# SunJiamei/LRP-ImageCaptioning

Measured on AMD Instinct MI355X. Metric: LRP heatmaps/sec (per predicted token) VGG16+adaptive-attn, 224x224, higher is better.
Workload: dtype bf16x3; 1 GPU; batch=32 synthetic 224x224 per GPU, VGG16 + adaptive-attention, LRP per-token heat-maps, 10 words/caption, V=10000 (BASELINE configs[1]); parallelism=image-sharded x1, RCCL weight broadcast, reverse_walk_precision=bf16x3, handles_per_gpu=2

## Files before the change

lrp-imagecaptioning_amd/csrc/common.h:

```cpp
#pragma once
#include <hip/hip_runtime.h>
#include <atomic>
#include <cstdarg>
#include <cstdio>
#include <cstdlib>
#include <string>
#include <vector>

#include "../../include/lrp_hip.h"

namespace lrp {

inline std::atomic<unsigned long long> g_launch_count{0};
#undef hipLaunchKernelGGL
#define hipLaunchKernelGGL(kernelName, numBlocks, numThreads, memPerBlock, streamId, ...)                  \
  do {                                                                                                    \
    ::lrp::g_launch_count.fetch_add(1, std::memory_order_relaxed);                                       \
    kernelName<<<(numBlocks), (numThreads), (memPerBlock), (streamId)>>>(__VA_ARGS__);                   \
  } while (0)

std::string& last_error_ref();

struct Switches {
  int conv_halo = 1;
  int conv_breg = 1;
  int conv_small = 1;
  int conv_mid = 1;
  int epi_fast = 1;
  int up2_pw = 1;
  int tile_order = 1;
  int fwd_emit = 1;
  int fwd_il = 1;
  int img_fused = 1;
  int up2_compact = 1;
  int img_fold = 1;
  int pool_fused = 1;
  int sparse_pool = 0;
  void load() {
    *this = Switches();
    auto rd = [](const char* name, int& v) { if (const char* e = getenv(name)) v = atoi(e); };
    rd("LRP_CONV_HALO", conv_halo); rd("LRP_CONV_BREG", conv_breg); rd("LRP_CONV_SMALL", conv_small);
    rd("LRP_CONV_MID", conv_mid); rd("LRP_EPI_FAST", epi_fast); rd("LRP_UP2_PW", up2_pw); rd("LRP_TILE_ORDER", tile_order);
    rd("LRP_FWD_EMIT", fwd_emit); rd("LRP_FWD_IL", fwd_il); rd("LRP_IMG_FUSED", img_fused); rd("LRP_UP2_COMPACT", up2_compact);
    rd("LRP_IMG_FOLD", img_fold); rd("LRP_SPARSE_POOL", sparse_pool); rd("LRP_POOL_FUSED", pool_fused);
  }
};
inline Switches& sw() {
  static Switches s = [] { Switches t; t.load(); return t; }();
  return s;
}

inline int fail(int code, const char* fmt, ...) {
  char buf[512];
  va_list ap;
  va_start(ap, fmt);
  vsnprintf(buf, sizeof(buf), fmt, ap);
  va_end(ap);
  last_error_ref() = buf;
  return code;
}

#define LRP_HIP_CHECK(expr)                                                                     \
  do {                                                                                          \
    hipError_t _e = (expr);                                                                     \
    if (_e != hipSuccess)                                                                       \
      return ::lrp::fail(LRP_ERR_HIP, "%s failed: %s (%s:%d)", #expr, hipGetErrorString(_e), \
                         __FILE__, __LINE__);                                                   \
  } while (0)

#define LRP_TRY(expr)         \
  do {                        \
    int _rc = (expr);         \
    if (_rc != LRP_OK) return _rc; \
  } while (0)

struct DevBuf {
  void* p = nullptr;
  size_t bytes = 0;
  bool owned = true;
  DevBuf() = default;
  DevBuf(const DevBuf&) = delete;
  DevBuf& operator=(const DevBuf&) = delete;
  DevBuf(DevBuf&& o) noexcept : p(o.p), bytes(o.bytes), owned(o.owned) { o.p = nullptr; o.bytes = 0; o.owned = true; }
  DevBuf& operator=(DevBuf&& o) noexcept {
    if (this != &o) { release(); p = o.p; bytes = o.bytes; owned = o.owned; o.p = nullptr; o.bytes = 0; o.owned = true; }
    return *this;
  }
  ~DevBuf() { release(); }
  void release() {
    if (p && owned) (void)hipFree(p);
    p = nullptr;
    bytes = 0;
    owned = true;
  }
  void view_of(const DevBuf& arena, size_t offset, size_t n) {
    release();
    p = static_cast<char*>(arena.p) + offset;
    bytes = n;
    owned = false;
  }
  int alloc(size_t n, int64_t* total) {
    release();
    if (n == 0) n = 16;
    hipError_t e = hipMalloc(&p, n);
    if (e != hipSuccess) {
      p = nullptr;
      (void)hipGetLastError();
      return fail(LRP_ERR_NOMEM, "device memory: hipMalloc(%zu bytes) failed: %s", n, hipGetErrorString(e));
    }
    bytes = n;
    if (total) *total += (int64_t)n;
    return LRP_OK;
  }
  template <typename T>
  T* as() const { return reinterpret_cast<T*>(p); }
};

}
```

lrp-imagecaptioning_amd/csrc/conv_sparse.h:

```cpp
#pragma once
#include "cnn_kernels.h"
#include "conv_igemm.h"

namespace lrp {

typedef __bf16 bf16x16 __attribute__((ext_vector_type(16)));
typedef unsigned u32x2 __attribute__((ext_vector_type(2)));

struct SparseArgs {
  const float* sc;
  const unsigned* idxp;
  const float* wsp;
  const float* gate;
  float* out;
  const int* row2img;
  int NB, Hp, Wp, C, N;
  int cols_t, m_tiles, n_tiles;
  int out_plain;
  int diag;
};

constexpr int SP_TW = 14, SP_TH = 18, SP_PITCH = SP_TW + 2;
constexpr int SP_NENT = (SP_TH + 2) * SP_PITCH;
constexpr int SP_PENT = SP_NENT + 1;
constexpr int SP_SUB = SP_PENT * 16;
constexpr int SP_ABUF = 3 * SP_SUB;
constexpr int SP_SUBPIECES = (SP_PENT + 63) / 64;
constexpr int SP_APIECES = 3 * SP_SUBPIECES;
constexpr int SP_ASLOTS = (SP_APIECES + 7) / 8;
constexpr int SP_BSTAGE = 32768, SP_NSTAGE = 4;
constexpr int SP_LDS = SP_NSTAGE * SP_BSTAGE + 2 * SP_ABUF + 128;
static_assert(SP_LDS <= 160 * 1024, "LDS");
static_assert(SP_PENT >= 64, "a DMA piece is 64 windows");

__host__ __device__ inline int sparse_slot_tap(int q, int group, int slot) {
  const int qy = q >> 1, qx = q & 1, sy = qy ? 1 : -1, sx = qx ? 1 : -1;
  int dy, dx;
  if (group == 0) { dy = (slot >> 1) - qy; dx = (slot & 1) - qx; }
  else if (group == 1) {
    if (slot < 2) { dy = slot - qy; dx = sx; }
    else if (slot == 2) { dy = sy; dx = sx; }
    else return -1;
  } else {
    if (slot < 2) { dy = sy; dx = slot - qx; }
    else return -1;
  }
  return 3 * (dy + 1) + (dx + 1);
}

__global__ __launch_bounds__(256) void conv_sparse_index_kernel(const unsigned char* __restrict__ pos, unsigned* __restrict__ idxp, size_t n_sets,
                                                                int HW, int C) {
  for (size_t i = (size_t)blockIdx.x * 256 + threadIdx.x; i < n_sets * 4; i += (size_t)gridDim.x * 256) {
    const int q = (int)(i & 3);
    const size_t set = i >> 2;
    const u32x2 pp = *reinterpret_cast<const u32x2*>(pos + set * 8);
    const unsigned qxm = (q & 1) ? 0x01010101u : 0u, qym = (q >> 1) ? 0x01010101u : 0u;
    unsigned word[4][2];
#pragma unroll
    for (int d = 0; d < 2; ++d) {
      const unsigned P = pp[d];
      const unsigned px = P & 0x01010101u, py = (P >> 1) & 0x01010101u;
      const unsigned mh = px ^ qxm, mv = py ^ qym;
      const unsigned nmh = mh ^ 0x01010101u, nmv = mv ^ 0x01010101u;
      word[0][d] = P | ((P ^ 0x01010101u) << 2);
      word[1][d] = py | nmh | (nmh << 1);
      word[2][d] = (0x02020202u | ((mh & mv) ^ 0x01010101u)) << 2;
      word[3][d] = (px & mv) | (nmv << 1) | 0x0C0C0C0Cu;
    }
    unsigned h0[4], h1[4];
#pragma unroll
    for (int pl = 0; pl < 4; ++pl) {
      const unsigned t0 = word[pl][0] | (word[pl][0] >> 4), t1 = word[pl][1] | (word[pl][1] >> 4);
      h0[pl] = (t0 & 0xFFu) | (((t0 >> 16) & 0xFFu) << 8);
      h1[pl] = (t1 & 0xFFu) | (((t1 >> 16) & 0xFFu) << 8);
    }
    const u32x4 iw = {h0[0] | (h0[1] << 16), h0[2] | (h0[3] << 16), h1[0] | (h1[1] << 16), h1[2] | (h1[3] << 16)};
    const int spw = C >> 3;
    const size_t win = set / spw;
    const int sw = (int)(set - win * spw), chunk = sw >> 1, s2 = sw & 1;
    const size_t img = win / HW, pix = win - img * HW;
    reinterpret_cast<u32x4*>(idxp)[((((img * 4 + q) * (C >> 4) + chunk) * HW + pix) << 1) + s2] = iw;
  }
}

__global__ __launch_bounds__(256) void conv_sparse_pairs_kernel(const float* __restrict__ sc, float* __restrict__ scp, size_t n_sets, int HW, int C) {
  for (size_t i = (size_t)blockIdx.x * 256 + threadIdx.x; i < n_sets; i += (size_t)gridDim.x * 256) {
    float v[8];
    *reinterpret_cast<f32x4*>(v) = *reinterpret_cast<const f32x4*>(sc + i * 8);
    *reinterpret_cast<f32x4*>(v + 4) = *reinterpret_cast<const f32x4*>(sc + i * 8 + 4);
    const int spw = C >> 3;
    const size_t win = i / spw;
    const int sw = (int)(i - win * spw), chunk = sw >> 1, s2 = sw & 1;
    const size_t n = win / HW, pix = win - n * HW;
    split8_store(v, scp + ((((n * (C >> 4) + chunk) * HW + pix) << 1) + s2) * 8);
  }
}

__global__ __launch_bounds__(256) void conv_sparse_relayout_kernel(const float* __restrict__ pairs, float* __restrict__ scp, size_t n_sets, int HW, int C) {
  for (size_t i = (size_t)blockIdx.x * 256 + threadIdx.x; i < n_sets; i += (size_t)gridDim.x * 256) {
    const u32x4 hi = *reinterpret_cast<const u32x4*>(pairs + i * 8), lo = *reinterpret_cast<const u32x4*>(pairs + i * 8 + 4);
    const int spw = C >> 3;
    const size_t win = i / spw;
    const int sw_ = (int)(i - win * spw), chunk = sw_ >> 1, s2 = sw_ & 1;
    const size_t n = win / HW, pix = win - n * HW;
    float* dst = scp + ((((n * (C >> 4) + chunk) * HW + pix) << 1) + s2) * 8;
    *reinterpret_cast<u32x4*>(dst) = hi;
    *reinterpret_cast<u32x4*>(dst + 4) = lo;
  }
}

__global__ __launch_bounds__(256) void conv_sparse_pack_kernel(const float* __restrict__ wb, float* __restrict__ wsp, int N, int C, int CPo,
                                                               int n_tiles) {
  const size_t total = (size_t)4 * n_tiles * (C / 16) * 6 * 2 * 2 * 256;
  for (size_t i = (size_t)blockIdx.x * 256 + threadIdx.x; i < total; i += (size_t)gridDim.x * 256) {
    const int col = (int)(i & 255);
    size_t r = i >> 8;
    const int part = (int)(r & 1); r >>= 1;
    const int half = (int)(r & 1); r >>= 1;
    const int step = (int)(r % 6); r /= 6;
    const int chunk = (int)(r % (C / 16)); r /= (C / 16);
    const int nt = (int)(r % n_tiles);
    const int q = (int)(r / n_tiles);
    const int ci = nt * 256 + col;
    bf16x8 hi, lo;
#pragma unroll
    for (int e = 0; e < 8; ++e) {
      const int k32 = 16 * half + 8 * part + e, cb = k32 >> 2, slot = k32 & 3;
      const int ch8 = 4 * ((cb >> 1) & 1) + 2 * (cb >> 2) + (cb & 1);
      const int co = chunk * 16 + (step & 1) * 8 + ch8;
      const int tap = sparse_slot_tap(q, step >> 1, slot);
      const float v = (tap >= 0 && ci < N && co < C) ? wb[(size_t)ci * 9 * CPo + (size_t)tap * CPo + co] : 0.f;
      hi[e] = (__bf16)v;
      lo[e] = (__bf16)(v - (float)hi[e]);
    }
    const size_t sbase = ((((size_t)q * n_tiles + nt) * (C / 16) + chunk) * 6 + step) * (SP_BSTAGE / 16);
    u32x4* dst = reinterpret_cast<u32x4*>(wsp);
    dst[sbase + ((0 * 2 + half) * 2 + part) * 256 + col] = __builtin_bit_cast(u32x4, hi);
    dst[sbase + ((1 * 2 + half) * 2 + part) * 256 + col] = __builtin_bit_cast(u32x4, lo);
  }
}

__global__ __launch_bounds__(512, 2) void conv_sparse_kernel(SparseArgs a) {
#if defined(__HIP_DEVICE_COMPILE__)
  __shared__ __attribute__((aligned(16))) unsigned char lds[SP_LDS];
  const int tid = threadIdx.x, lane = tid & 63, wave = tid >> 6, wm = wave >> 2, wn = wave & 3;
  const int l31 = lane & 31, half = lane >> 5;
  const int per_class = a.m_tiles * a.n_tiles;
  const int q = blockIdx.x / per_class, rem = blockIdx.x - q * per_class;
  const int nt = rem / a.m_tiles, mt = rem - nt * a.m_tiles;
  const int qy = q >> 1, qx = q & 1, sy = qy ? 1 : -1, sx = qx ? 1 : -1;
  const int tyt = mt / a.cols_t, txt = mt - tyt * a.cols_t;
  const int Y0 = tyt * SP_TH, x0 = txt * SP_TW;
  const int Hp = a.Hp, Wp = a.Wp, C = a.C, N = a.N, H = 2 * Hp, W = 2 * Wp;
  const int nys = a.NB * Hp;
  const int n0 = nt * 256;
  const float inv_Hp = 1.0f / (float)Hp;
  auto divmod = [](int x, int d, float inv, int& qq, int& r) {
    qq = (int)(((float)x + 0.5f) * inv);
    r = x - qq * d;
    if (r < 0) { --qq; r += d; } else if (r >= d) { ++qq; r -= d; }
  };
  unsigned char* Bs = lds;
  unsigned char* As = lds + SP_NSTAGE * SP_BSTAGE;

  auto chunk0 = [&](int e) { return e * 16 + half * 8; };
  int e_own[4], e_h[4], e_v[4], e_d[4];
#pragma unroll
  for (int i = 0; i < 4; ++i) {
    const int r = (wm * 4 + i) * 32 + l31;
    const int ty = r / SP_TW, tx = r - ty * SP_TW;
    const int Ys = Y0 + ty, wx = x0 + tx;
    int n_, wy;
    divmod(Ys, Hp, inv_Hp, n_, wy);
    const bool ok = r < SP_TH * SP_TW && Ys < nys && wx < Wp;
    const bool okh = ok && wx + sx >= 0 && wx + sx < Wp, okv = ok && wy + sy >= 0 && wy + sy < Hp;
    const int e = (ty + 1) * SP_PITCH + tx + 1;
    e_own[i] = chunk0(ok ? e : SP_NENT);
    e_h[i] = chunk0(okh ? e + sx : SP_NENT);
    e_v[i] = chunk0(okv ? e + sy * SP_PITCH : SP_NENT);
    e_d[i] = chunk0(okh && okv ? e + sy * SP_PITCH + sx : SP_NENT);
  }

  typedef __attribute__((address_space(3))) void* lptr_t;
  constexpr int RSRC_FLAGS = 0x00020000;
  const int nchunks = C >> 4, nsteps = nchunks * 6;
  const __amdgpu_buffer_rsrc_t rsB = __builtin_amdgcn_make_buffer_rsrc(
      (void*)(reinterpret_cast<const unsigned char*>(a.wsp) + ((size_t)q * a.n_tiles + nt) * (size_t)nsteps * SP_BSTAGE), 0, nsteps * SP_BSTAGE, RSRC_FLAGS);
  const int wave_s = __builtin_amdgcn_readfirstlane(wave);
  auto fire_b = [&](int step, int stage) {
#pragma unroll
    for (int p = 0; p < 4; ++p)
      __builtin_amdgcn_raw_ptr_buffer_load_lds(rsB, (lptr_t)(Bs + stage * SP_BSTAGE + (wave_s * 4 + p) * 1024), 16, lane * 16,
                                               step * SP_BSTAGE + (wave_s * 4 + p) * 1024, 0, 0);
  };

  int* imgtab = reinterpret_cast<int*>(As + 2 * SP_ABUF);
  if (tid < SP_TH + 2) {
    const int Ys = Y0 - 1 + tid;
    int n_, wy;
    divmod(Ys >= 0 && Ys < nys ? Ys : 0, Hp, inv_Hp, n_, wy);
    imgtab[tid] = a.row2img ? a.row2img[n_] : n_;
  }
  const __amdgpu_buffer_rsrc_t rsS = __builtin_amdgcn_make_buffer_rsrc((void*)a.sc, 0, 0x7FFFFFFF, RSRC_FLAGS);
  const __amdgpu_buffer_rsrc_t rsI = __builtin_amdgcn_make_buffer_rsrc((void*)a.idxp, 0, 0x7FFFFFFF, RSRC_FLAGS);
  constexpr int OOB = (int)0x80000000;
  auto fire_a = [&](int slot, int set8, int abuf) {
    int wv = wave_s, ln = lane;
    asm volatile("" : "+s"(wv), "+v"(ln));
    int pj = wv + 8 * slot;
    if (pj >= SP_APIECES) pj = SP_APIECES - 1;
    const int pl = pj / SP_SUBPIECES, jp = pj - pl * SP_SUBPIECES;
    const int first = jp * 64 < SP_PENT - 64 ? jp * 64 : SP_PENT - 64;
    const int e = first + ln;
    const int hy = e >> 4, hx = e & 15;
    const int Ys = Y0 - 1 + hy, wx = x0 - 1 + hx;
    const bool ok = e < SP_NENT && Ys >= 0 && Ys < nys && wx >= 0 && wx < Wp;
    int n_, wy;
    divmod(ok ? Ys : 0, Hp, inv_Hp, n_, wy);
    const int chunk = set8 >> 1, s = set8 & 1;
    int vo;
    if (pl < 2) {
      vo = ((((n_ * (C >> 4) + chunk) * Hp + wy) * Wp + wx) << 6) + s * 32 + pl * 16;
    } else {
      const int img = imgtab[ok ? hy : 0];
      vo = (((((img * 4 + q) * (C >> 4) + chunk) * Hp + wy) * Wp + wx) << 5) + s * 16;
    }
    __builtin_amdgcn_raw_ptr_buffer_load_lds(pl < 2 ? rsS : rsI, (lptr_t)(As + abuf * SP_ABUF + pl * SP_SUB + first * 16), 16, ok ? vo : OOB,
                                             0, 0, 0);
  };
  auto fire_set = [&](int set8, int abuf) {
#pragma unroll
    for (int sl = 0; sl < SP_ASLOTS; ++sl) fire_a(sl, set8, abuf);
  };

  const int nsteps2 = nchunks * 6;
  auto bsrc = [&](int chunk, int t6) { return chunk * 6 + 2 * (t6 % 3) + t6 / 3; };
  __syncthreads();
  fire_set(0, 0);
  if (nchunks * 2 > 1) fire_set(1, 1);
  fire_b(bsrc(0, 0), 0);
  fire_b(bsrc(0, 1), 1);
  asm volatile("s_waitcnt vmcnt(0)" ::: "memory");
  __syncthreads();

  f32x16 acc[4][2];
#pragma unroll
  for (int i = 0; i < 4; ++i)
#pragma unroll
    for (int j = 0; j < 2; ++j)
#pragma unroll
      for (int r = 0; r < 16; ++r) acc[i][j][r] = 0.f;

  const int bcol = (wn * 64 + l31) * 16 + half * 8192;
  auto expand = [](u32x2 x) -> bf16x8 {
    const u32x4 r = {x[0] & 0xFFFFu, x[0] >> 16, x[1] & 0xFFFFu, x[1] >> 16};
    return __builtin_bit_cast(bf16x8, r);
  };
  auto pairup = [](u32x2 h, u32x2 d) -> bf16x8 {
    const u32x4 r = {__builtin_amdgcn_perm(d[0], h[0], 0x05040100u), __builtin_amdgcn_perm(d[0], h[0], 0x07060302u),
                     __builtin_amdgcn_perm(d[1], h[1], 0x05040100u), __builtin_amdgcn_perm(d[1], h[1], 0x07060302u)};
    return __builtin_bit_cast(bf16x8, r);
  };
  auto ld8 = [](const unsigned char* p) { return *reinterpret_cast<const u32x2*>(p); };
  auto ld2 = [](const unsigned char* p) { return (unsigned)*reinterpret_cast<const unsigned short*>(p); };
  struct BF { bf16x16 h[2], l[2]; };
  auto load_b = [&](BF& b, const unsigned char* Bb) {
#pragma unroll
    for (int j = 0; j < 2; ++j) {
      const unsigned char* bp = Bb + j * 512;
      const bf16x8 h0 = *reinterpret_cast<const bf16x8*>(bp), h1 = *reinterpret_cast<const bf16x8*>(bp + 4096);
      const bf16x8 l0 = *reinterpret_cast<const bf16x8*>(bp + 16384), l1 = *reinterpret_cast<const bf16x8*>(bp + 16384 + 4096);
      b.h[j] = __builtin_shufflevector(h0, h1, 0, 1, 2, 3, 4, 5, 6, 7, 8, 9, 10, 11, 12, 13, 14, 15);
      b.l[j] = __builtin_shufflevector(l0, l1, 0, 1, 2, 3, 4, 5, 6, 7, 8, 9, 10, 11, 12, 13, 14, 15);
    }
  };
  auto kstep = [&](const unsigned char* Ab, int grp, const BF& b) {
    const unsigned char* Ah = Ab;
    const unsigned char* Al = Ab + SP_SUB;
    const unsigned char* Ai = Ab + 2 * SP_SUB;
#pragma unroll
    for (int i = 0; i < 4; ++i) {
      bf16x8 vh, vl;
      int ix;
      if (grp == 1) {
        const int oh = e_h[i], od = e_d[i];
        vh = pairup(ld8(Ah + oh), ld8(Ah + od));
        vl = pairup(ld8(Al + oh), ld8(Al + od));
        ix = (int)(ld2(Ai + oh + 2) | ld2(Ai + od + 4));
      } else {
        const int oo = grp == 0 ? e_own[i] : e_v[i];
        vh = expand(ld8(Ah + oo));
        vl = expand(ld8(Al + oo));
        ix = (int)ld2(Ai + oo + (grp == 0 ? 0 : 6));
      }
#pragma unroll
      for (int j = 0; j < 2; ++j) {
        acc[i][j] = __builtin_amdgcn_smfmac_f32_32x32x32_bf16(vl, b.h[j], acc[i][j], ix, 0, 0);
        acc[i][j] = __builtin_amdgcn_smfmac_f32_32x32x32_bf16(vh, b.l[j], acc[i][j], ix, 0, 0);
        acc[i][j] = __builtin_amdgcn_smfmac_f32_32x32x32_bf16(vh, b.h[j], acc[i][j], ix, 0, 0);
      }
    }
  };

  for (int chunk = 0; chunk < nchunks; ++chunk) {
    const bool next_chunk = chunk + 1 < nchunks;
#pragma unroll
    for (int ss = 0; ss < 3; ++ss) {
      const int t0 = 2 * ss, t1 = 2 * ss + 1;
      const int st0 = chunk * 6 + t0;
      if (st0 + 2 < nsteps2) {
        const int nc = ss == 2 ? chunk + 1 : chunk, nt0 = (t0 + 2) % 6;
        fire_b(bsrc(nc, nt0), (st0 + 2) & 3);
        fire_b(bsrc(nc, nt0 + 1), (st0 + 3) & 3);
      }
      if (ss == 2 && next_chunk) fire_set(2 * chunk + 2, 0);
      if (ss == 0 && chunk > 0) fire_set(2 * chunk + 1, 1);
      BF b0, b1;
      load_b(b0, Bs + (st0 & 3) * SP_BSTAGE + bcol);
      load_b(b1, Bs + ((st0 + 1) & 3) * SP_BSTAGE + bcol);
      kstep(As + (t0 / 3) * SP_ABUF, t0 % 3, b0);
      kstep(As + (t1 / 3) * SP_ABUF, t1 % 3, b1);
      asm volatile("s_waitcnt vmcnt(0) lgkmcnt(0)\n\ts_barrier" ::: "memory");
    }
  }

  float* Cs = reinterpret_cast<float*>(lds);
#pragma unroll
  for (int sl = 0; sl < 4; ++sl) {
    f32x4 g[4][2];
    bool ok4[4];
    size_t off4[4];
#pragma unroll
    for (int p = 0; p < 4; ++p) {
      const int item = tid + p * 512, row = item >> 5, cg = item & 31;
      const int R = sl * 64 + row;
      const int ty = R / SP_TW, tx = R - ty * SP_TW;
      const int Ys = Y0 + ty, wx = x0 + tx;
      int n_, wy;
      divmod(Ys < nys ? Ys : 0, Hp, inv_Hp, n_, wy);
      const int col = n0 + cg * 8;
      ok4[p] = R < SP_TH * SP_TW && Ys < nys && wx < Wp && col < N && !((a.diag & 1) && (row | cg | sl));
      const int y = 2 * wy + qy, x = 2 * (wx < Wp ? wx : 0) + qx;
      const int img = a.row2img ? a.row2img[n_] : n_;
      const size_t goff = (((size_t)img * H + y) * W + x) * N + (col < N ? col : 0);
      off4[p] = (((size_t)n_ * H + y) * W + x) * N + (col < N ? col : 0);
      g[p][0] = *reinterpret_cast<const f32x4*>(a.gate + goff);
      g[p][1] = *reinterpret_cast<const f32x4*>(a.gate + goff + 4);
    }
    if (sl) __syncthreads();
    if (wm == (sl >> 1)) {
      float* cw = Cs + (4 * half) * 256 + wn * 64 + l31;
#pragma unroll
      for (int ii = 0; ii < 2; ++ii)
#pragma unroll
        for (int r = 0; r < 16; ++r)
#pragma unroll
          for (int j = 0; j < 2; ++j) cw[(ii * 32 + (r & 3) + 8 * (r >> 2)) * 256 + j * 32] = acc[2 * (sl & 1) + ii][j][r];
    }
    __syncthreads();
#pragma unroll
    for (int p = 0; p < 4; ++p) {
      if (!ok4[p]) continue;
      const int item = tid + p * 512, row = item >> 5, cg = item & 31;
      const f32x4 c0 = *reinterpret_cast<const f32x4*>(Cs + row * 256 + cg * 8), c1 = *reinterpret_cast<const f32x4*>(Cs + row * 256 + cg * 8 + 4);
      float r[8];
#pragma unroll
      for (int e = 0; e < 4; ++e) { r[e] = c0[e] * g[p][0][e]; r[4 + e] = c1[e] * g[p][1][e]; }
      float* dst = a.out + off4[p];
      if (a.out_plain) {
        *reinterpret_cast<f32x4*>(dst) = *reinterpret_cast<const f32x4*>(r);
        *reinterpret_cast<f32x4*>(dst + 4) = *reinterpret_cast<const f32x4*>(r + 4);
      } else {
        split8_store(r, dst);
      }
    }
  }
#endif
}

inline size_t conv_sparse_weight_floats(int N, int C) { return (size_t)4 * ((N + 255) / 256) * (C / 16) * 6 * (SP_BSTAGE / 4); }
inline bool conv_sparse_supports(int N, int C, int Hp, int Wp) { return N % 256 == 0 && C % 16 == 0 && Hp >= 1 && Wp >= 1; }

inline hipError_t conv_sparse_pack(const float* wb_dev, float* wsp_dev, int N, int C, hipStream_t st) {
  const int n_tiles = (N + 255) / 256;
  const size_t total = (size_t)4 * n_tiles * (C / 16) * 6 * 2 * 2 * 256;
  hipLaunchKernelGGL(conv_sparse_pack_kernel, dim3((unsigned)((total + 255) / 256)), dim3(256), 0, st, wb_dev, wsp_dev, N, C, conv_cinp(C), n_tiles);
  return hipGetLastError();
}

inline size_t conv_sparse_index_words(int images, int Hp, int Wp, int C) { return (size_t)images * Hp * Wp * (C / 8) * 4 * 4; }
inline hipError_t conv_sparse_index(const unsigned char* pos_dev, unsigned* idxp_dev, int images, int Hp, int Wp, int C, hipStream_t st) {
  const size_t n_sets = (size_t)images * Hp * Wp * (C / 8);
  hipLaunchKernelGGL(conv_sparse_index_kernel, dim3(stream_grid(n_sets * 4)), dim3(256), 0, st, pos_dev, idxp_dev, n_sets, Hp * Wp, C);
  return hipGetLastError();
}
inline hipError_t conv_sparse_pairs(const float* sc_dev, float* scp_dev, int NB, int Hp, int Wp, int C, hipStream_t st) {
  const size_t n_sets = (size_t)NB * Hp * Wp * (C / 8);
  hipLaunchKernelGGL(conv_sparse_pairs_kernel, dim3(stream_grid(n_sets)), dim3(256), 0, st, sc_dev, scp_dev, n_sets, Hp * Wp, C);
  return hipGetLastError();
}

inline hipError_t conv_sparse_launch(SparseArgs a, hipStream_t st) {
  if (!conv_sparse_supports(a.N, a.C, a.Hp, a.Wp) || !a.sc || !a.idxp || !a.wsp || !a.gate || !a.out) return hipErrorInvalidValue;
  if (a.NB <= 0) return hipSuccess;
  a.cols_t = (a.Wp + SP_TW - 1) / SP_TW;
  a.n_tiles = a.N / 256;
  a.m_tiles = ((a.NB * a.Hp + SP_TH - 1) / SP_TH) * a.cols_t;
  hipLaunchKernelGGL(conv_sparse_kernel, dim3(4 * a.m_tiles * a.n_tiles), dim3(512), 0, st, a);
  return hipGetLastError();
}

}
```

lrp-imagecaptioning_amd/csrc/encoder.h:

```cpp
#pragma once
#include <algorithm>
#include <functional>
#include <memory>
#include <string>
#include <vector>

#include "cnn_kernels.h"
#include "common.h"
#include "conv_igemm.h"
#include "conv_sparse.h"
#include "f16_operand.h"

namespace lrp {

struct ConvLayer {
  std::string name;
  int cin = 0, cout = 0, H = 0, W = 0;
  bool pool_after = false;
  bool have_w = false, have_b = false;
  DevBuf w_fwd;
  DevBuf w_fwd_a;
  DevBuf w_fwd_zs;
  DevBuf w_fwd_as;
  DevBuf w_fwd_h;
// ... 566 lines not shown
          hipLaunchKernelGGL(gate_kernel, dim3(stream_grid(n / 4)), dim3(256), 0, side,
                             reinterpret_cast<const f32x4*>(keep_acts ? L.Akeep.as<float>() : L.G.as<float>()),
                             reinterpret_cast<const f32x4*>(bufZ.as<float>()), L.G.as<f32x4>(), n / 4);
        LRP_HIP_CHECK(hipGetLastError());
      }
      LRP_HIP_CHECK(hipEventRecord(ev_gates, side));
      gates_pending = true;
    }
    encoded = B;
    features_only = false;
    return LRP_OK;
  }

  int full_gate(int li, hipStream_t st) {
    ConvLayer& L = layers[li];
    if (!L.pool_after || L.gfull_epoch == encode_epoch) return LRP_OK;
    if (!L.Gc.p || L.gc_epoch != encode_epoch) return fail(LRP_ERR_STATE, "no pool gate of layer %d for this encode", li);
    const size_t n8 = (size_t)encoded * (L.H / 2) * (L.W / 2) * (L.cout / 8);
    hipLaunchKernelGGL(pool_gate_expand_kernel, dim3(stream_grid(n8)), dim3(256), 0, st, L.Gc.as<float>(), L.Gpos.as<unsigned char>(),
                       L.G.as<float>(), encoded, L.H, L.W, L.cout);
    LRP_HIP_CHECK(hipGetLastError());
    L.gfull_epoch = encode_epoch;
    return LRP_OK;
  }

  int explain(int n, const int* row2img_dev, const float* R_feat_dev, float* R_img_dev, hipStream_t st, int walk = 0,
              const std::function<int(int, const float*)>* layer_hook = nullptr) {
    const int* r2i_host = row2img_host;
    row2img_host = nullptr;
    if (n < 1 || n > max_tokens) return fail(LRP_ERR_INVALID, "n=%d outside [1,%d]", n, max_tokens);
    if (walk < 0 || walk > 3) return fail(LRP_ERR_INVALID, "unknown walk %d", walk);
    if (encoded < 1 || features_only) return fail(LRP_ERR_STATE, "lrp_encode_images must run before the CNN explain");
    if (gates_pending) LRP_HIP_CHECK(hipStreamWaitEvent(st, ev_gates, 0));
    const ConvLayer& T = layers.back();
    float* S = s0.as<float>();
    float* Snext = s1.as<float>();
    bool split = prec == PREC_BF16X3 && walk == 0;
    bool hook_split = prec == PREC_BF16X3 && walk == 1 && layer_hook != nullptr;
    for (const ConvLayer& L : layers)
      if (L.cout & 7) split = hook_split = false;
    for (size_t li = 1; li < layers.size(); ++li)
      if (!layers[li].w_bwd_full_s.p) hook_split = false;
    const bool f16 = split && walk_f16 && img_fused();
    if (f16) {
      const size_t cnt = (layers.size() + 1) * (size_t)max_tokens;
      if (!tok_exp.p) {
        int64_t dummy = 0;
        LRP_TRY(tok_exp.alloc(cnt * sizeof(int), &dummy));
        LRP_TRY(tok_max.alloc(cnt * sizeof(unsigned), &dummy));
        LRP_TRY(tok_fac.alloc((size_t)max_tokens * sizeof(float), &dummy));
      }
      LRP_HIP_CHECK(hipMemsetAsync(tok_max.p, 0, cnt * sizeof(unsigned), st));
    }
    auto lev_exp = [&](int lev) { return tok_exp.as<int>() + (size_t)lev * max_tokens; };
    auto lev_max = [&](int lev) { return tok_max.as<unsigned>() + (size_t)lev * max_tokens; };
    const int run_prec = f16 ? PREC_F16X2 : (split || hook_split) ? PREC_BF16X3 : PREC_FP32;
    if (walk != 0) {
      const size_t per4 = T.act_elems() / 4;
      hipLaunchKernelGGL(grad_top_kernel, dim3(stream_grid((size_t)n * per4)), dim3(256), 0, st,
                         reinterpret_cast<const f32x4*>(R_feat_dev), feat.as<f32x4>(), row2img_dev,
                         reinterpret_cast<f32x4*>(S), n, per4, walk == 3 ? 1 : 0);
      LRP_HIP_CHECK(hipGetLastError());
    } else if (f16) {
      const int top = (int)layers.size() - 1;
      hipLaunchKernelGGL(top_divide_f16_kernel, dim3(n), dim3(256), 0, st, R_feat_dev, ztop.as<float>(), row2img_dev, S,
                         T.act_elems() / 8, lev_exp(top), lev_max(top));
      LRP_HIP_CHECK(hipGetLastError());
    } else if (split) {
      const size_t per8 = T.act_elems() / 8;
      hipLaunchKernelGGL(top_divide_split_kernel, dim3(stream_grid((size_t)n * per8)), dim3(256), 0, st, R_feat_dev,
                         ztop.as<float>(), row2img_dev, S, n, per8);
      LRP_HIP_CHECK(hipGetLastError());
    } else {
      const size_t per4 = T.act_elems() / 4;
      hipLaunchKernelGGL(top_divide_kernel, dim3(stream_grid((size_t)n * per4)), dim3(256), 0, st,
                         reinterpret_cast<const f32x4*>(R_feat_dev), ztop.as<f32x4>(), row2img_dev,
                         reinterpret_cast<f32x4*>(S), n, per4);
      LRP_HIP_CHECK(hipGetLastError());
    }
    const bool up2_on = sw().up2_compact != 0;
    bool pairs_in = false;
    int fold_tw = 0, fold_th = 0;
    const bool fold_on = sw().img_fold != 0;
    auto writes_pairs = [&](int li) {
      const ConvLayer& P = layers[li - 1];
      if (!P.pool_after || !up2_on || !split || f16 || walk != 0 || layer_hook || li < 2 || (P.cout & 7) || !P.Gc.p ||
          P.gc_epoch != encode_epoch)
        return false;
      const bool cons_fold = li == 2 && fold_on && img_fused() && !layers[0].pool_after && P.cin == 64 && conv_cinp(P.cout) <= 64 &&
                             layers[0].w_bwd_s.p != nullptr && conv_takes_breg(P.cin, P.H, P.W, P.w_bwd_frag.p != nullptr);
      return cons_fold || conv_takes_pw(P.cin, n, P.H, P.W);
    };
    for (int li = (int)layers.size() - 1; li >= 0; --li) {
      const ConvLayer& L = layers[li];
      if (layer_hook) {
        LRP_TRY((*layer_hook)(li, S));
        if (li == 0) return LRP_OK;
      }
      ConvArgs ca{};
      ca.in = S; ca.NB = n; ca.H = L.H; ca.W = L.W; ca.Cin = L.cout; ca.CinP = conv_cinp(L.cout); ca.taps = 9;
      if (hook_split) {
        const size_t n8 = (size_t)n * L.act_elems() / 8;
        hipLaunchKernelGGL(split_copy_kernel, dim3(stream_grid(n8)), dim3(256), 0, st, S, bufXs.as<float>(), n8);
        LRP_HIP_CHECK(hipGetLastError());
        ca.in = bufXs.as<float>();
        ca.out_plain = 1;
      }
      ca.wpk = hook_split ? L.w_bwd_full_s.as<float>() : walk != 0 ? L.w_bwd_full.as<float>() : f16 ? L.w_bwd_h.as<float>()
               : split ? L.w_bwd_s.as<float>() : L.w_bwd.as<float>();
      ca.wpk_frag = f16 ? L.w_bwd_frag_h.as<float>() : (split && walk == 0) ? L.w_bwd_frag.as<float>() : nullptr;
      if (f16) {
        hipLaunchKernelGGL(tok_scale_kernel, dim3((n + 255) / 256), dim3(256), 0, st, lev_max(li), lev_exp(li),
                           L.wbs.as<float>(), tok_fac.as<float>(), li > 0 ? lev_exp(li - 1) : (int*)nullptr,
                           n, li == 0 ? 1 : 0);
        LRP_HIP_CHECK(hipGetLastError());
        ca.tok_fac = tok_fac.as<float>();
        if (li > 0) ca.tok_max_out = lev_max(li - 1);
      }
      ca.row2img = row2img_dev;
      ca.order = L.order.get(); ca.row2img_host = r2i_host;
      ca.gate_binary = walk != 0; ca.relu_out = walk == 3;
      int epi;
      if (li == 0 && img_fused()) {
        ca.taps = 1; ca.N = IMG_T_COLS; ca.out = R_img_dev; ca.ximg = images.as<float>();
        ca.img_mode = walk == 0 ? 0 : walk == 2 ? 2 : 1;
        epi = EPI_IMG_STENCIL;
      } else if (li == 0) {
        ca.NB = n * L.H * L.W; ca.H = 1; ca.W = 1; ca.taps = 1;
        ca.N = IMG_T_COLS; ca.out = Snext; epi = EPI_STORE;
      } else {
        const ConvLayer& P = layers[li - 1];
        ca.N = L.cin; ca.aux = P.G.as<float>(); ca.out = Snext;
        epi = P.pool_after ? EPI_MUL_UP2 : EPI_MUL;
        if (li == 1 && fold_on && split && !f16 && walk == 0 && !layer_hook && img_fused() && !P.pool_after && L.cin == 64 &&
            P.w_bwd_s.p && conv_takes_breg(L.cin, L.H, L.W, L.w_bwd_frag.p != nullptr)) {
          int hr_ = 0;
          (void)conv_halo_geom(128, L.H, L.W, fold_tw, fold_th, hr_);
          ca.img_w = P.w_bwd_s.as<float>(); ca.img_part = Snext; ca.out = nullptr;
        }
        if (pairs_in && sw().sparse_pool && L.w_sp.p && L.idx_epoch == encode_epoch && !P.pool_after && split && !f16 && walk == 0 &&
            !layer_hook && sp_scp.p) {
          const int Hp = L.H / 2, Wp = L.W / 2;
          const size_t n_sets = (size_t)n * Hp * Wp * (L.cout / 8);
          ProfileRec pr{};
          if (profile) { (void)hipEventCreate(&pr.e0); (void)hipEventCreate(&pr.e1); (void)hipEventRecord(pr.e0, st); }
          hipLaunchKernelGGL(conv_sparse_relayout_kernel, dim3(stream_grid(n_sets)), dim3(256), 0, st, S, sp_scp.as<float>(), n_sets, Hp * Wp, L.cout);
          LRP_HIP_CHECK(hipGetLastError());
          SparseArgs sa{};
          sa.sc = sp_scp.as<float>(); sa.idxp = L.idxp.as<unsigned>(); sa.wsp = L.w_sp.as<float>(); sa.gate = P.G.as<float>(); sa.out = Snext;
          sa.row2img = row2img_dev; sa.NB = n; sa.Hp = Hp; sa.Wp = Wp; sa.C = L.cout; sa.N = L.cin;
          LRP_HIP_CHECK(conv_sparse_launch(sa, st));
          if (profile) {
            (void)hipEventRecord(pr.e1, st);
            pr.flop = 2.0 * (double)n * L.H * L.W * 9.0 * L.cout * L.cin;
            prof.push_back(pr);
          }
          pairs_in = false;
          float* t = S; S = Snext; Snext = t;
          continue;
        }
        if (pairs_in) {
          ca.up2_src = S; ca.up2_pairs = 1; ca.up2_gpos = L.Gpos.as<unsigned char>();
          pairs_in = false;
        }
        if (writes_pairs(li)) {
          epi = EPI_MUL; ca.aux = P.Gc.as<float>();
          pairs_in = true;
        }
      }
      ProfileRec pr{};
      if (profile) {
        (void)hipEventCreate(&pr.e0); (void)hipEventCreate(&pr.e1);
        (void)hipEventRecord(pr.e0, st);
      }
      const int terms = f16 && two_term(li) ? 5 : 7;
      if (epi == EPI_MUL_UP2) LRP_TRY(full_gate(li - 1, st));
      LRP_HIP_CHECK(conv_launch(epi, ca, st, run_prec, terms));
      if (profile) {
        (void)hipEventRecord(pr.e1, st);
        pr.flop = 2.0 * (double)n * L.H * L.W * 9.0 * L.cout * (li == 0 ? 6 : L.cin);
        prof.push_back(pr);
      }
      if (ca.img_part) {
        const ConvLayer& L0 = layers[0];
        ProfileRec p2{};
        if (profile) {
          (void)hipEventCreate(&p2.e0); (void)hipEventCreate(&p2.e1);
          (void)hipEventRecord(p2.e0, st);
        }
        hipLaunchKernelGGL(img_partial_sum_kernel, dim3(stream_grid((size_t)n * L0.H * L0.W)), dim3(256), 0, st, ca.img_part, images.as<float>(),
                           row2img_dev, R_img_dev, n, L0.H, L0.W, fold_th, fold_tw, (L0.W + fold_tw - 1) / fold_tw, 0);
        LRP_HIP_CHECK(hipGetLastError());
        if (profile) {
          (void)hipEventRecord(p2.e1, st);
          p2.flop = 2.0 * (double)n * L0.H * L0.W * 9.0 * L0.cout * 6;
          prof.push_back(p2);
        }
        return LRP_OK;
      }
      float* t = S; S = Snext; Snext = t;
    }
    if (!img_fused()) {
      const ConvLayer& L0 = layers[0];
      hipLaunchKernelGGL(img_stencil_kernel, dim3(stream_grid((size_t)n * L0.H * L0.W)), dim3(256), 0, st, S,
                         images.as<float>(), row2img_dev, R_img_dev, n, L0.H, L0.W, walk == 0 ? 0 : walk == 2 ? 2 : 1);
      LRP_HIP_CHECK(hipGetLastError());
    }
    return LRP_OK;
  }

  int profile_records(int cap, double* ms_out, double* flop_out, int* n_out) {
    int k = 0;
    for (ProfileRec& p : prof) {
      float t = 0.f;
      const bool ok = hipEventSynchronize(p.e1) == hipSuccess && hipEventElapsedTime(&t, p.e0, p.e1) == hipSuccess;
      if (ok && k < cap) { ms_out[k] = t; flop_out[k] = p.flop; ++k; }
      (void)hipEventDestroy(p.e0); (void)hipEventDestroy(p.e1);
    }
    prof.clear();
    *n_out = k;
    return LRP_OK;
  }

  int profile_query(int64_t* launches, double* ms, double* flop) {
// ... 16 lines not shown
```

Baseline: 10040 heatmaps/s.

## Enable sparse pooled-conv path by default with templated small-tile variant

```diff
diff --git a/lrp-imagecaptioning_amd/csrc/common.h b/lrp-imagecaptioning_amd/csrc/common.h
--- a/lrp-imagecaptioning_amd/csrc/common.h
+++ b/lrp-imagecaptioning_amd/csrc/common.h
@@ -35,7 +35,7 @@
   int up2_compact = 1;
   int img_fold = 1;
   int pool_fused = 1;
-  int sparse_pool = 0;
+  int sparse_pool = 1;
   void load() {
     *this = Switches();
     auto rd = [](const char* name, int& v) { if (const char* e = getenv(name)) v = atoi(e); };
diff --git a/lrp-imagecaptioning_amd/csrc/conv_sparse.h b/lrp-imagecaptioning_amd/csrc/conv_sparse.h
--- a/lrp-imagecaptioning_amd/csrc/conv_sparse.h
+++ b/lrp-imagecaptioning_amd/csrc/conv_sparse.h
@@ -20,18 +20,36 @@
   int diag;
 };
 
-constexpr int SP_TW = 14, SP_TH = 18, SP_PITCH = SP_TW + 2;
-constexpr int SP_NENT = (SP_TH + 2) * SP_PITCH;
-constexpr int SP_PENT = SP_NENT + 1;
-constexpr int SP_SUB = SP_PENT * 16;
-constexpr int SP_ABUF = 3 * SP_SUB;
-constexpr int SP_SUBPIECES = (SP_PENT + 63) / 64;
-constexpr int SP_APIECES = 3 * SP_SUBPIECES;
-constexpr int SP_ASLOTS = (SP_APIECES + 7) / 8;
-constexpr int SP_BSTAGE = 32768, SP_NSTAGE = 4;
-constexpr int SP_LDS = SP_NSTAGE * SP_BSTAGE + 2 * SP_ABUF + 128;
-static_assert(SP_LDS <= 160 * 1024, "LDS");
-static_assert(SP_PENT >= 64, "a DMA piece is 64 windows");
+constexpr int SP_TW = 14, SP_PITCH = SP_TW + 2;
+constexpr int SP_BPACK = 32768, SP_NSTAGE = 4;
+
+template <int WMW_, int WNW_, int MI_, int NJ_, int TH_>
+struct SparseTile {
+  static constexpr int WMW = WMW_, WNW = WNW_, MI = MI_, NJ = NJ_, TH = TH_;
+  static constexpr int NW = WMW * WNW, NT = 64 * NW;
+  static constexpr int BM = WMW * MI * 32, BN = WNW * NJ * 32;
+  static constexpr int NENT = (TH + 2) * SP_PITCH;
+  static constexpr int PENT = NENT + 1;
+  static constexpr int SUB = PENT * 16;
+  static constexpr int ABUF = 3 * SUB;
+  static constexpr int SUBPIECES = (PENT + 63) / 64;
+  static constexpr int APIECES = 3 * SUBPIECES;
+  static constexpr int ASLOTS = (APIECES + NW - 1) / NW;
+  static constexpr int PLANE = BN * 16;
+  static constexpr int BSTAGE = 8 * PLANE;
+  static constexpr int BPIECES = BSTAGE / 1024 / NW;
+  static constexpr int NSLAB = BM / 64;
+  static constexpr int EPI_P = 64 * (BN / 8) / NT;
+  static constexpr int LDS = SP_NSTAGE * BSTAGE + 2 * ABUF + 128;
+  static_assert(TH * SP_TW <= BM && BM % 64 == 0 && 256 % BN == 0, "tile");
+  static_assert(BPIECES * NW * 1024 == BSTAGE && EPI_P * NT == 64 * (BN / 8), "pieces");
+  static_assert(SP_NSTAGE * BSTAGE >= 64 * BN * 4, "the epilogue's C slab lies in the B stages");
+  static_assert((TH + 2) * 4 <= 128, "image table");
+  static_assert(LDS <= 160 * 1024, "LDS");
+  static_assert(PENT >= 64, "a DMA piece is 64 windows");
+};
+typedef SparseTile<2, 4, 4, 2, 18> SparseTileLarge;
+typedef SparseTile<2, 2, 1, 2, 4> SparseTileSmall;
 
 __host__ __device__ inline int sparse_slot_tap(int q, int group, int slot) {
   const int qy = q >> 1, qx = q & 1, sy = qy ? 1 : -1, sx = qx ? 1 : -1;
@@ -133,27 +151,31 @@
       hi[e] = (__bf16)v;
       lo[e] = (__bf16)(v - (float)hi[e]);
     }
-    const size_t sbase = ((((size_t)q * n_tiles + nt) * (C / 16) + chunk) * 6 + step) * (SP_BSTAGE / 16);
+    const size_t sbase = ((((size_t)q * n_tiles + nt) * (C / 16) + chunk) * 6 + step) * (SP_BPACK / 16);
     u32x4* dst = reinterpret_cast<u32x4*>(wsp);
     dst[sbase + ((0 * 2 + half) * 2 + part) * 256 + col] = __builtin_bit_cast(u32x4, hi);
     dst[sbase + ((1 * 2 + half) * 2 + part) * 256 + col] = __builtin_bit_cast(u32x4, lo);
   }
 }
 
-__global__ __launch_bounds__(512, 2) void conv_sparse_kernel(SparseArgs a) {
+template <class TL>
+__global__ __launch_bounds__(TL::NT, 2) void conv_sparse_kernel(SparseArgs a) {
 #if defined(__HIP_DEVICE_COMPILE__)
-  __shared__ __attribute__((aligned(16))) unsigned char lds[SP_LDS];
-  const int tid = threadIdx.x, lane = tid & 63, wave = tid >> 6, wm = wave >> 2, wn = wave & 3;
+  constexpr int MI = TL::MI, NJ = TL::NJ, NW = TL::NW, NT = TL::NT, BN = TL::BN, TH = TL::TH;
+  constexpr int NENT = TL::NENT, PENT = TL::PENT, SUB = TL::SUB, ABUF = TL::ABUF, BSTAGE = TL::BSTAGE, PLANE = TL::PLANE;
+  __shared__ __attribute__((aligned(16))) unsigned char lds[TL::LDS];
+  const int tid = threadIdx.x, lane = tid & 63, wave = tid >> 6, wm = wave / TL::WNW, wn = wave % TL::WNW;
   const int l31 = lane & 31, half = lane >> 5;
   const int per_class = a.m_tiles * a.n_tiles;
   const int q = blockIdx.x / per_class, rem = blockIdx.x - q * per_class;
   const int nt = rem / a.m_tiles, mt = rem - nt * a.m_tiles;
   const int qy = q >> 1, qx = q & 1, sy = qy ? 1 : -1, sx = qx ? 1 : -1;
   const int tyt = mt / a.cols_t, txt = mt - tyt * a.cols_t;
-  const int Y0 = tyt * SP_TH, x0 = txt * SP_TW;
+  const int Y0 = tyt * TH, x0 = txt * SP_TW;
   const int Hp = a.Hp, Wp = a.Wp, C = a.C, N = a.N, H = 2 * Hp, W = 2 * Wp;
   const int nys = a.NB * Hp;
-  const int n0 = nt * 256;
+  const int n0 = nt * BN;
+  const int nt256 = n0 >> 8, ncol0 = n0 & 255;
   const float inv_Hp = 1.0f / (float)Hp;
   auto divmod = [](int x, int d, float inv, int& qq, int& r) {
     qq = (int)(((float)x + 0.5f) * inv);
@@ -161,41 +183,44 @@
     if (r < 0) { --qq; r += d; } else if (r >= d) { ++qq; r -= d; }
   };
   unsigned char* Bs = lds;
-  unsigned char* As = lds + SP_NSTAGE * SP_BSTAGE;
+  unsigned char* As = lds + SP_NSTAGE * BSTAGE;
 
   auto chunk0 = [&](int e) { return e * 16 + half * 8; };
-  int e_own[4], e_h[4], e_v[4], e_d[4];
-#pragma unroll
-  for (int i = 0; i < 4; ++i) {
-    const int r = (wm * 4 + i) * 32 + l31;
+  int e_own[MI], e_h[MI], e_v[MI], e_d[MI];
+#pragma unroll
+  for (int i = 0; i < MI; ++i) {
+    const int r = (wm * MI + i) * 32 + l31;
     const int ty = r / SP_TW, tx = r - ty * SP_TW;
     const int Ys = Y0 + ty, wx = x0 + tx;
     int n_, wy;
     divmod(Ys, Hp, inv_Hp, n_, wy);
-    const bool ok = r < SP_TH * SP_TW && Ys < nys && wx < Wp;
+    const bool ok = r < TH * SP_TW && Ys < nys && wx < Wp;
     const bool okh = ok && wx + sx >= 0 && wx + sx < Wp, okv = ok && wy + sy >= 0 && wy + sy < Hp;
     const int e = (ty + 1) * SP_PITCH + tx + 1;
-    e_own[i] = chunk0(ok ? e : SP_NENT);
-    e_h[i] = chunk0(okh ? e + sx : SP_NENT);
-    e_v[i] = chunk0(okv ? e + sy * SP_PITCH : SP_NENT);
-    e_d[i] = chunk0(okh && okv ? e + sy * SP_PITCH + sx : SP_NENT);
+    e_own[i] = chunk0(ok ? e : NENT);
+    e_h[i] = chunk0(okh ? e + sx : NENT);
+    e_v[i] = chunk0(okv ? e + sy * SP_PITCH : NENT);
+    e_d[i] = chunk0(okh && okv ? e + sy * SP_PITCH + sx : NENT);
   }
 
   typedef __attribute__((address_space(3))) void* lptr_t;
   constexpr int RSRC_FLAGS = 0x00020000;
   const int nchunks = C >> 4, nsteps = nchunks * 6;
   const __amdgpu_buffer_rsrc_t rsB = __builtin_amdgcn_make_buffer_rsrc(
-      (void*)(reinterpret_cast<const unsigned char*>(a.wsp) + ((size_t)q * a.n_tiles + nt) * (size_t)nsteps * SP_BSTAGE), 0, nsteps * SP_BSTAGE, RSRC_FLAGS);
+      (void*)(reinterpret_cast<const unsigned char*>(a.wsp) + ((size_t)q * (N >> 8) + nt256) * (size_t)nsteps * SP_BPACK), 0, nsteps * SP_BPACK, RSRC_FLAGS);
   const int wave_s = __builtin_amdgcn_readfirstlane(wave);
   auto fire_b = [&](int step, int stage) {
 #pragma unroll
-    for (int p = 0; p < 4; ++p)
-      __builtin_amdgcn_raw_ptr_buffer_load_lds(rsB, (lptr_t)(Bs + stage * SP_BSTAGE + (wave_s * 4 + p) * 1024), 16, lane * 16,
-                                               step * SP_BSTAGE + (wave_s * 4 + p) * 1024, 0, 0);
-  };
-
-  int* imgtab = reinterpret_cast<int*>(As + 2 * SP_ABUF);
-  if (tid < SP_TH + 2) {
+    for (int p = 0; p < TL::BPIECES; ++p) {
+      const int pc = wave_s * TL::BPIECES + p;
+      const int plane = pc / (BN / 64), sub = pc - plane * (BN / 64);
+      __builtin_amdgcn_raw_ptr_buffer_load_lds(rsB, (lptr_t)(Bs + stage * BSTAGE + pc * 1024), 16, lane * 16,
+                                               step * SP_BPACK + plane * 4096 + (ncol0 + sub * 64) * 16, 0, 0);
+    }
+  };
+
+  int* imgtab = reinterpret_cast<int*>(As + 2 * ABUF);
+  if (tid < TH + 2) {
     const int Ys = Y0 - 1 + tid;
     int n_, wy;
     divmod(Ys >= 0 && Ys < nys ? Ys : 0, Hp, inv_Hp, n_, wy);
@@ -207,14 +232,14 @@
   auto fire_a = [&](int slot, int set8, int abuf) {
     int wv = wave_s, ln = lane;
     asm volatile("" : "+s"(wv), "+v"(ln));
-    int pj = wv + 8 * slot;
-    if (pj >= SP_APIECES) pj = SP_APIECES - 1;
-    const int pl = pj / SP_SUBPIECES, jp = pj - pl * SP_SUBPIECES;
-    const int first = jp * 64 < SP_PENT - 64 ? jp * 64 : SP_PENT - 64;
+    int pj = wv + NW * slot;
+    if (pj >= TL::APIECES) pj = TL::APIECES - 1;
+    const int pl = pj / TL::SUBPIECES, jp = pj - pl * TL::SUBPIECES;
+    const int first = jp * 64 < PENT - 64 ? jp * 64 : PENT - 64;
     const int e = first + ln;
     const int hy = e >> 4, hx = e & 15;
     const int Ys = Y0 - 1 + hy, wx = x0 - 1 + hx;
-    const bool ok = e < SP_NENT && Ys >= 0 && Ys < nys && wx >= 0 && wx < Wp;
+    const bool ok = e < NENT && Ys >= 0 && Ys < nys && wx >= 0 && wx < Wp;
     int n_, wy;
     divmod(ok ? Ys : 0, Hp, inv_Hp, n_, wy);
     const int chunk = set8 >> 1, s = set8 & 1;
@@ -225,12 +250,12 @@
       const int img = imgtab[ok ? hy : 0];
       vo = (((((img * 4 + q) * (C >> 4) + chunk) * Hp + wy) * Wp + wx) << 5) + s * 16;
     }
-    __builtin_amdgcn_raw_ptr_buffer_load_lds(pl < 2 ? rsS : rsI, (lptr_t)(As + abuf * SP_ABUF + pl * SP_SUB + first * 16), 16, ok ? vo : OOB,
+    __builtin_amdgcn_raw_ptr_buffer_load_lds(pl < 2 ? rsS : rsI, (lptr_t)(As + abuf * ABUF + pl * SUB + first * 16), 16, ok ? vo : OOB,
                                              0, 0, 0);
   };
   auto fire_set = [&](int set8, int abuf) {
 #pragma unroll
-    for (int sl = 0; sl < SP_ASLOTS; ++sl) fire_a(sl, set8, abuf);
+    for (int sl = 0; sl < TL::ASLOTS; ++sl) fire_a(sl, set8, abuf);
   };
 
   const int nsteps2 = nchunks * 6;
@@ -243,15 +268,15 @@
   asm volatile("s_waitcnt vmcnt(0)" ::: "memory");
   __syncthreads();
 
-  f32x16 acc[4][2];
-#pragma unroll
-  for (int i = 0; i < 4; ++i)
-#pragma unroll
-    for (int j = 0; j < 2; ++j)
+  f32x16 acc[MI][NJ];
+#pragma unroll
+  for (int i = 0; i < MI; ++i)
+#pragma unroll
+    for (int j = 0; j < NJ; ++j)
 #pragma unroll
       for (int r = 0; r < 16; ++r) acc[i][j][r] = 0.f;
 
-  const int bcol = (wn * 64 + l31) * 16 + half * 8192;
+  const int bcol = (wn * (NJ * 32) + l31) * 16 + half * (2 * PLANE);
   auto expand = [](u32x2 x) -> bf16x8 {
     const u32x4 r = {x[0] & 0xFFFFu, x[0] >> 16, x[1] & 0xFFFFu, x[1] >> 16};
     return __builtin_bit_cast(bf16x8, r);
@@ -263,23 +288,23 @@
   };
   auto ld8 = [](const unsigned char* p) { return *reinterpret_cast<const u32x2*>(p); };
   auto ld2 = [](const unsigned char* p) { return (unsigned)*reinterpret_cast<const unsigned short*>(p); };
-  struct BF { bf16x16 h[2], l[2]; };
+  struct BF { bf16x16 h[NJ], l[NJ]; };
   auto load_b = [&](BF& b, const unsigned char* Bb) {
 #pragma unroll
-    for (int j = 0; j < 2; ++j) {
+    for (int j = 0; j < NJ; ++j) {
       const unsigned char* bp = Bb + j * 512;
-      const bf16x8 h0 = *reinterpret_cast<const bf16x8*>(bp), h1 = *reinterpret_cast<const bf16x8*>(bp + 4096);
-      const bf16x8 l0 = *reinterpret_cast<const bf16x8*>(bp + 16384), l1 = *reinterpret_cast<const bf16x8*>(bp + 16384 + 4096);
+      const bf16x8 h0 = *reinterpret_cast<const bf16x8*>(bp), h1 = *reinterpret_cast<const bf16x8*>(bp + PLANE);
+      const bf16x8 l0 = *reinterpret_cast<const bf16x8*>(bp + 4 * PLANE), l1 = *reinterpret_cast<const bf16x8*>(bp + 4 * PLANE + PLANE);
       b.h[j] = __builtin_shufflevector(h0, h1, 0, 1, 2, 3, 4, 5, 6, 7, 8, 9, 10, 11, 12, 13, 14, 15);
       b.l[j] = __builtin_shufflevector(l0, l1, 0, 1, 2, 3, 4, 5, 6, 7, 8, 9, 10, 11, 12, 13, 14, 15);
     }
   };
   auto kstep = [&](const unsigned char* Ab, int grp, const BF& b) {
     const unsigned char* Ah = Ab;
-    const unsigned char* Al = Ab + SP_SUB;
-    const unsigned char* Ai = Ab + 2 * SP_SUB;
-#pragma unroll
-    for (int i = 0; i < 4; ++i) {
+    const unsigned char* Al = Ab + SUB;
+    const unsigned char* Ai = Ab + 2 * SUB;
+#pragma unroll
+    for (int i = 0; i < MI; ++i) {
       bf16x8 vh, vl;
       int ix;
       if (grp == 1) {
@@ -294,7 +319,7 @@
         ix = (int)ld2(Ai + oo + (grp == 0 ? 0 : 6));
       }
 #pragma unroll
-      for (int j = 0; j < 2; ++j) {
+      for (int j = 0; j < NJ; ++j) {
         acc[i][j] = __builtin_amdgcn_smfmac_f32_32x32x32_bf16(vl, b.h[j], acc[i][j], ix, 0, 0);
         acc[i][j] = __builtin_amdgcn_smfmac_f32_32x32x32_bf16(vh, b.l[j], acc[i][j], ix, 0, 0);
         acc[i][j] = __builtin_amdgcn_smfmac_f32_32x32x32_bf16(vh, b.h[j], acc[i][j], ix, 0, 0);
@@ -316,30 +341,30 @@
       if (ss == 2 && next_chunk) fire_set(2 * chunk + 2, 0);
       if (ss == 0 && chunk > 0) fire_set(2 * chunk + 1, 1);
       BF b0, b1;
-      load_b(b0, Bs + (st0 & 3) * SP_BSTAGE + bcol);
-      load_b(b1, Bs + ((st0 + 1) & 3) * SP_BSTAGE + bcol);
-      kstep(As + (t0 / 3) * SP_ABUF, t0 % 3, b0);
-      kstep(As + (t1 / 3) * SP_ABUF, t1 % 3, b1);
+      load_b(b0, Bs + (st0 & 3) * BSTAGE + bcol);
+      load_b(b1, Bs + ((st0 + 1) & 3) * BSTAGE + bcol);
+      kstep(As + (t0 / 3) * ABUF, t0 % 3, b0);
+      kstep(As + (t1 / 3) * ABUF, t1 % 3, b1);
       asm volatile("s_waitcnt vmcnt(0) lgkmcnt(0)\n\ts_barrier" ::: "memory");
     }
   }
 
   float* Cs = reinterpret_cast<float*>(lds);
 #pragma unroll
-  for (int sl = 0; sl < 4; ++sl) {
-    f32x4 g[4][2];
-    bool ok4[4];
-    size_t off4[4];
-#pragma unroll
-    for (int p = 0; p < 4; ++p) {
-      const int item = tid + p * 512, row = item >> 5, cg = item & 31;
+  for (int sl = 0; sl < TL::NSLAB; ++sl) {
+    f32x4 g[TL::EPI_P][2];
+    bool ok4[TL::EPI_P];
+    size_t off4[TL::EPI_P];
+#pragma unroll
+    for (int p = 0; p < TL::EPI_P; ++p) {
+      const int item = tid + p * NT, row = item / (BN / 8), cg = item % (BN / 8);
       const int R = sl * 64 + row;
       const int ty = R / SP_TW, tx = R - ty * SP_TW;
       const int Ys = Y0 + ty, wx = x0 + tx;
       int n_, wy;
       divmod(Ys < nys ? Ys : 0, Hp, inv_Hp, n_, wy);
       const int col = n0 + cg * 8;
-      ok4[p] = R < SP_TH * SP_TW && Ys < nys && wx < Wp && col < N && !((a.diag & 1) && (row | cg | sl));
+      ok4[p] = R < TH * SP_TW && Ys < nys && wx < Wp && col < N && !((a.diag & 1) && (row | cg | sl));
       const int y = 2 * wy + qy, x = 2 * (wx < Wp ? wx : 0) + qx;
       const int img = a.row2img ? a.row2img[n_] : n_;
       const size_t goff = (((size_t)img * H + y) * W + x) * N + (col < N ? col : 0);
@@ -348,21 +373,23 @@
       g[p][1] = *reinterpret_cast<const f32x4*>(a.gate + goff + 4);
     }
     if (sl) __syncthreads();
-    if (wm == (sl >> 1)) {
-      float* cw = Cs + (4 * half) * 256 + wn * 64 + l31;
-#pragma unroll
-      for (int ii = 0; ii < 2; ++ii)
+    float* cw = Cs + (4 * half) * BN + wn * (NJ * 32) + l31;
+#pragma unroll
+    for (int ii = 0; ii < 2; ++ii) {
+      const int f = 2 * sl + ii;
+      if (wm == f / MI) {
 #pragma unroll
         for (int r = 0; r < 16; ++r)
 #pragma unroll
-          for (int j = 0; j < 2; ++j) cw[(ii * 32 + (r & 3) + 8 * (r >> 2)) * 256 + j * 32] = acc[2 * (sl & 1) + ii][j][r];
+          for (int j = 0; j < NJ; ++j) cw[(ii * 32 + (r & 3) + 8 * (r >> 2)) * BN + j * 32] = acc[f % MI][j][r];
+      }
     }
     __syncthreads();
 #pragma unroll
-    for (int p = 0; p < 4; ++p) {
+    for (int p = 0; p < TL::EPI_P; ++p) {
       if (!ok4[p]) continue;
-      const int item = tid + p * 512, row = item >> 5, cg = item & 31;
-      const f32x4 c0 = *reinterpret_cast<const f32x4*>(Cs + row * 256 + cg * 8), c1 = *reinterpret_cast<const f32x4*>(Cs + row * 256 + cg * 8 + 4);
+      const int item = tid + p * NT, row = item / (BN / 8), cg = item % (BN / 8);
+      const f32x4 c0 = *reinterpret_cast<const f32x4*>(Cs + row * BN + cg * 8), c1 = *reinterpret_cast<const f32x4*>(Cs + row * BN + cg * 8 + 4);
       float r[8];
 #pragma unroll
       for (int e = 0; e < 4; ++e) { r[e] = c0[e] * g[p][0][e]; r[4 + e] = c1[e] * g[p][1][e]; }
@@ -378,7 +405,7 @@
 #endif
 }
 
-inline size_t conv_sparse_weight_floats(int N, int C) { return (size_t)4 * ((N + 255) / 256) * (C / 16) * 6 * (SP_BSTAGE / 4); }
+inline size_t conv_sparse_weight_floats(int N, int C) { return (size_t)4 * ((N + 255) / 256) * (C / 16) * 6 * (SP_BPACK / 4); }
 inline bool conv_sparse_supports(int N, int C, int Hp, int Wp) { return N % 256 == 0 && C % 16 == 0 && Hp >= 1 && Wp >= 1; }
 
 inline hipError_t conv_sparse_pack(const float* wb_dev, float* wsp_dev, int N, int C, hipStream_t st) {
@@ -400,14 +427,28 @@
   return hipGetLastError();
 }
 
+constexpr long CONV_SPARSE_SMALL_BLOCKS = 96L;
+inline long conv_sparse_large_blocks(int NB, int Hp, int Wp, int N) {
+  return 4L * ((NB * Hp + SparseTileLarge::TH - 1) / SparseTileLarge::TH) * ((Wp + SP_TW - 1) / SP_TW) * (N / SparseTileLarge::BN);
+}
+inline bool conv_sparse_small_grid(int NB, int Hp, int Wp, int N) {
+  return conv_small_tile_on() && conv_sparse_large_blocks(NB, Hp, Wp, N) <= CONV_SPARSE_SMALL_BLOCKS;
+}
+
+template <class TL>
+inline hipError_t conv_sparse_launch_tile(SparseArgs a, hipStream_t st) {
+  a.cols_t = (a.Wp + SP_TW - 1) / SP_TW;
+  a.n_tiles = a.N / TL::BN;
+  a.m_tiles = ((a.NB * a.Hp + TL::TH - 1) / TL::TH) * a.cols_t;
+  hipLaunchKernelGGL(conv_sparse_kernel<TL>, dim3(4 * a.m_tiles * a.n_tiles), dim3(TL::NT), 0, st, a);
+  return hipGetLastError();
+}
+
 inline hipError_t conv_sparse_launch(SparseArgs a, hipStream_t st) {
   if (!conv_sparse_supports(a.N, a.C, a.Hp, a.Wp) || !a.sc || !a.idxp || !a.wsp || !a.gate || !a.out) return hipErrorInvalidValue;
   if (a.NB <= 0) return hipSuccess;
-  a.cols_t = (a.Wp + SP_TW - 1) / SP_TW;
-  a.n_tiles = a.N / 256;
-  a.m_tiles = ((a.NB * a.Hp + SP_TH - 1) / SP_TH) * a.cols_t;
-  hipLaunchKernelGGL(conv_sparse_kernel, dim3(4 * a.m_tiles * a.n_tiles), dim3(512), 0, st, a);
-  return hipGetLastError();
-}
-
-}
+  const bool small = (a.diag & 4) ? true : (a.diag & 2) ? false : conv_sparse_small_grid(a.NB, a.Hp, a.Wp, a.N);
+  return small ? conv_sparse_launch_tile<SparseTileSmall>(a, st) : conv_sparse_launch_tile<SparseTileLarge>(a, st);
+}
+
+}
diff --git a/lrp-imagecaptioning_amd/csrc/encoder.h b/lrp-imagecaptioning_amd/csrc/encoder.h
--- a/lrp-imagecaptioning_amd/csrc/encoder.h
+++ b/lrp-imagecaptioning_amd/csrc/encoder.h
@@ -672,11 +672,18 @@
     bool pairs_in = false;
     int fold_tw = 0, fold_th = 0;
     const bool fold_on = sw().img_fold != 0;
+    auto sparse_consumer = [&](int lc) {
+      if (lc < 1) return false;
+      const ConvLayer& Lc = layers[lc];
+      return sw().sparse_pool && Lc.w_sp.p && Lc.idxp.p && Lc.idx_epoch == encode_epoch && !layers[lc - 1].pool_after && split && !f16 &&
+             walk == 0 && !layer_hook && sp_scp.p != nullptr;
+    };
     auto writes_pairs = [&](int li) {
       const ConvLayer& P = layers[li - 1];
-      if (!P.pool_after || !up2_on || !split || f16 || walk != 0 || layer_hook || li < 2 || (P.cout & 7) || !P.Gc.p ||
-          P.gc_epoch != encode_epoch)
+      if (!P.pool_after || !split || f16 || walk != 0 || layer_hook || li < 2 || (P.cout & 7) || !P.Gc.p || P.gc_epoch != encode_epoch)
         return false;
+      if (sparse_consumer(li - 1)) return true;
+      if (!up2_on) return false;
       const bool cons_fold = li == 2 && fold_on && img_fused() && !layers[0].pool_after && P.cin == 64 && conv_cinp(P.cout) <= 64 &&
                              layers[0].w_bwd_s.p != nullptr && conv_takes_breg(P.cin, P.H, P.W, P.w_bwd_frag.p != nullptr);
       return cons_fold || conv_takes_pw(P.cin, n, P.H, P.W);
@@ -728,8 +735,7 @@
           (void)conv_halo_geom(128, L.H, L.W, fold_tw, fold_th, hr_);
           ca.img_w = P.w_bwd_s.as<float>(); ca.img_part = Snext; ca.out = nullptr;
         }
-        if (pairs_in && sw().sparse_pool && L.w_sp.p && L.idx_epoch == encode_epoch && !P.pool_after && split && !f16 && walk == 0 &&
-            !layer_hook && sp_scp.p) {
+        if (pairs_in && sparse_consumer(li)) {
           const int Hp = L.H / 2, Wp = L.W / 2;
           const size_t n_sets = (size_t)n * Hp * Wp * (L.cout / 8);
           ProfileRec pr{};
diff --git a/profiles/sparse_forms.py b/profiles/sparse_forms.py
--- /dev/null
+++ b/profiles/sparse_forms.py
@@ -0,0 +1,35 @@
+#!/usr/bin/env python3
+import os
+import sys
+import time
+
+import numpy as np
+import torch
+
+sys.path.insert(0, os.path.dirname(os.path.dirname(os.path.abspath(__file__))))
+from lrp_imagecaptioning_amd.engine import op_conv_pool_sparse
+
+SHAPES = {"block4_conv3": (14, 14, 512, 512), "block3_conv3": (28, 28, 256, 256)}
+for name, (Hp, Wp, Cin, Cout) in SHAPES.items():
+    for NB in (1, 3, 5, 10, 15, 20, 30, 40, 60, 90):
+        rs = np.random.RandomState(0)
+        g = torch.Generator(device="cuda").manual_seed(1)
+        sc = torch.randn((NB, Hp, Wp, Cout), device="cuda", generator=g)
+        pos = torch.randint(0, 4, (NB, Hp, Wp, Cout), device="cuda", generator=g, dtype=torch.uint8)
+        w = np.abs(rs.standard_normal((3, 3, Cin, Cout)) / np.sqrt(9 * Cout)).astype(np.float32)
+        gate = torch.rand((NB, 2 * Hp, 2 * Wp, Cin), device="cuda", generator=g)
+        res = {}
+        for form, bit in (("large", 2), ("small", 4)):
+            op_conv_pool_sparse(sc, pos, w, gate, reps=3 | (bit << 8))
+            best = 1e9
+            for _ in range(3):
+                torch.cuda.synchronize()
+                t0 = time.perf_counter()
+                op_conv_pool_sparse(sc, pos, w, gate, reps=1 | (bit << 8))
+                t1 = time.perf_counter()
+                op_conv_pool_sparse(sc, pos, w, gate, reps=101 | (bit << 8))
+                t2 = time.perf_counter()
+                best = min(best, ((t2 - t1) - (t1 - t0)) / 100 * 1e6)
+            res[form] = best
+        blocks = 4 * ((NB * Hp + 17) // 18) * ((Wp + 13) // 14) * (Cin // 256)
+        print("%s NB=%d large-form workgroups %d: large %.1f us, small %.1f us" % (name, NB, blocks, res["large"], res["small"]), flush=True)
```

Result: faster. 10210 heatmaps/s (median of 6 runs) (+1.7%).
